# AdaptiveCity/deepdish

Measured on AMD Instinct MI355X. Metric: end-to-end frames/sec (detect+encode+track) at 640x480, higher is better.
Workload: dtype i8 (reference: uint8); encoder f16; 1 GPU; SSD-MobileNet-v1 uint8-quantised (300x300) + MARS-64x32x3 + deep_sort on synthetic 640x480 BGR frames, ~20 synthetic detections/frame (BASELINE.json configs[1]); streams_per_gpu=3072, worker_threads_per_gpu=2, parallelism=independent streams, 3072 per GPU in 2 worker groups, weights=seeded synthetic (seed 1234)

## Files before the change

### deepdish_amd/_lib.py

```python
import ctypes
import os
from ctypes import c_int, c_int64, c_double, c_float, c_void_p, c_char_p, POINTER

HERE = os.path.dirname(os.path.abspath(__file__))
LIB_PATH = os.environ.get('DD_LIB') or os.path.join(HERE, 'libdeepdish_hip.so')

P = c_void_p


class DeepDishHipError(RuntimeError):
    pass


SIGNATURES = {
    'dd_last_error': [],
    'dd_version': [],
    'dd_ctx_create': [c_int, POINTER(P)],
    'dd_ctx_destroy': [P],
    'dd_ctx_stream': [P, POINTER(P)],
    'dd_ctx_sync': [P],
    'dd_kf_initiate': [P, P, P, P, P, c_int, P],
    'dd_kf_predict': [P, P, P, P, c_int, P],
    'dd_kf_project': [P, P, P, P, c_int, P, P, P],
    'dd_kf_update': [P, P, P, P, P, c_int, P],
    'dd_kf_gate': [P, P, P, P, c_int, P, c_int, c_int, P, P],
    'dd_iou_cost': [P, P, P, c_int, P, c_int, P, P],
    'dd_cosine_nn_cost': [P, P, P, c_int, P, c_int, P, P],
    'dd_euclidean_nn_cost': [P, P, P, c_int, P, c_int, P, P],
    'dd_nms': [P, P, P, c_int, c_double, P, P, P],
    'dd_nms_ssd': [P, P, P, c_int, c_double, P, P, P],
    'dd_lsap_host': [P, c_int, c_int, P, P],
    'dd_pyset_difference_order_host': [P, c_int, P, c_int, P, POINTER(c_int)],
    'dd_lsap_batch': [P, P, P, P, P, c_int, P, P],
    'dd_match_cascade': [P, c_int, P, P, c_int, c_int, P, P, c_double, c_double, c_int, P, POINTER(c_int), P, POINTER(c_int), P,
                         POINTER(c_int)],
    'dd_tracker_create': [P, c_double, c_double, c_int, c_int, c_int, c_int, c_int, POINTER(P)],
    'dd_tracker_create_metric': [P, c_int, c_double, c_double, c_int, c_int, c_int, c_int, c_int, POINTER(P)],
    'dd_tracker_destroy': [P],
    'dd_tracker_predict': [P],
    'dd_tracker_update': [P, P, P, c_int, c_int],
    'dd_tracker_count': [P, c_int, POINTER(c_int)],
    'dd_tracker_read': [P, c_int, P, P, P],
    'dd_tracker_track_update': [P, c_int64, P, P, c_int],
    'dd_tracker_track_predict': [P, c_int64],
    'dd_tracker_track_set': [P, c_int64, c_int, c_int],
    'dd_tracker_remove': [P, P, c_int],
    'dd_tracker_next_id': [P, POINTER(c_int64)],
    'dd_tracker_last_cost': [P, P, P, c_int, POINTER(c_int), POINTER(c_int)],
    'dd_tracker_last_matches': [P, P, c_int, POINTER(c_int)],
    'dd_tracker_set_association': [P, c_int],
    'dd_tracker_association_stats': [P, POINTER(ctypes.c_longlong), POINTER(ctypes.c_longlong), POINTER(ctypes.c_longlong),
                                     POINTER(ctypes.c_longlong)],
    'dd_crop_resize': [P, P, c_int, c_int, P, c_int, c_int, c_int, P, P, P],
    'dd_crop_resize_f64': [P, P, c_int, c_int, P, c_int, c_int, c_int, P, P, P],
    'dd_fake_encode': [P, P, c_int, c_int, P, P],
    'dd_resize_lanczos': [P, P, c_int, c_int, c_int, c_int, P, c_int, c_int, P],
    'dd_resize_lanczos_batch': [P, P, c_int, c_int, c_int, c_int, c_int, P, c_int, c_int, P],
    'dd_resize_lanczos_plan': [P, c_int, c_int, c_int, c_int, c_int, c_int, c_int, P, P, P, POINTER(c_int), POINTER(c_int), POINTER(c_int),
                               POINTER(c_int)],
    'dd_letterbox_geometry': [c_int, c_int, c_int, c_int, POINTER(c_int), POINTER(c_int), POINTER(c_int), POINTER(c_int)],
    'dd_resize_lanczos_letterbox': [P, P, c_int, c_int, c_int, c_int, c_int, P, c_int, c_int, c_int, P],
    'dd_resize_lanczos_letterbox_plan': [P, c_int, c_int, c_int, c_int, c_int, c_int, c_int, POINTER(c_int), POINTER(c_int)],
    'dd_resize_bilinear': [P, P, c_int, c_int, c_int, P, c_int, c_int, P],
    'dd_yuv420_to_bgr': [P, P, c_int, c_int, c_int, c_int, c_int, c_int64, c_int64, P, P],
    'dd_yuv422_to_bgr': [P, P, c_int, c_int, c_int, c_int, c_int, c_int64, P, P],
    'dd_ingest_create': [P, c_int, c_int, c_int, c_int, c_int, c_int, c_int, P],
    'dd_ingest_create_format': [P, c_int, c_int, c_int, c_int, c_int, c_int, c_int, c_int, P],
    'dd_ingest_create_jpeg': [P, c_int, c_int, c_int, c_int, c_int, c_int, c_int, c_int64, P],
    'dd_ingest_jpeg_put': [P, c_int, c_int, P, c_int64],
    'dd_ingest_status': [P, c_int, P],
    'dd_ingest_destroy': [P],
    'dd_ingest_host_slot': [P, c_int, P, P],
    'dd_ingest_submit': [P, c_int],
    'dd_ingest_wait_uploaded': [P, c_int],
    'dd_ingest_acquire': [P, c_int, P, P],
    'dd_ingest_release': [P, c_int, P],
    'dd_mog2_create': [P, c_int, c_int, c_int, c_int, c_double, c_int, POINTER(P)],
    'dd_mog2_destroy': [P],
    'dd_mog2_state': [P, c_int, P, P, P, P],
    'dd_mog2_apply': [P, P, c_double, P, P, P],
    'dd_mask_box_count': [P, P, c_int, c_int, c_int, P, P, c_int, P, P],
    'dd_net_create': [P, P, c_int, P, c_int64, c_int, POINTER(P)],
    'dd_net_create_shared': [P, P, c_int, P, c_int64, c_int, POINTER(P)],
    'dd_net_activation_bytes': [P, POINTER(c_int64)],
    'dd_net_destroy': [P],
    'dd_net_forward': [P, P, c_int, P],
    'dd_net_output': [P, c_int, POINTER(P), POINTER(c_int), POINTER(c_int), POINTER(c_int), POINTER(c_int),
                      POINTER(c_int)],
    'dd_net_use_graph': [P, c_int],
    'dd_net_input_size': [P, POINTER(c_int), POINTER(c_int)],
    'dd_net_max_batch': [P, POINTER(c_int)],
    'dd_net_last_batch': [P, POINTER(c_int)],
    'dd_net_read': [P, c_int, c_int, P, c_int, P],
    'dd_net_profile': [P, c_int],
    'dd_net_profile_read': [P, P, c_int, POINTER(c_int)],
    'dd_net_op_launches': [P, P, c_int, POINTER(c_int)],
    'dd_net_op_variants': [P, P, c_int, POINTER(c_int)],
    'dd_netq_dwpw_fits': [c_int, c_int, c_int, c_int, c_int, c_int, POINTER(c_int)],
    'dd_ssd_postprocess': [P, P, P, c_int, c_int, c_int, c_float, c_float, P, P, P, P, P],
    'dd_ssd_decode': [P, P, P, c_int, c_int, c_float, P, P, P, P, c_int, P],
    'dd_ssd_postprocess_decoded': [P, P, P, P, P, c_int, c_int, c_float, c_float, P, P, P, P, c_int, P],
    'dd_ssd_regular_nms_decoded': [P, P, P, c_int, c_int, c_int, c_int, c_int, c_int, c_float, c_float, P, P, P, P, c_int, P],
    'dd_ssd_postprocess_regular': [P, P, P, c_int, c_int, c_int, c_int, c_float, c_float, P, P, P, P, c_int, P],
    'dd_ssd_postprocess_regular_u8': [P, P, P, c_int, P, P, P, c_int, c_int, c_int, c_int, c_float, c_float, P, P, P, P, c_int, P],
    'dd_net_ssd_heads_u8': [P, POINTER(P), POINTER(P), POINTER(c_int), POINTER(P), P, POINTER(c_int), POINTER(c_int)],
    'dd_net_ssd_decode': [P, P, c_int, c_float, c_int],
    'dd_net_ssd_decoded': [P, POINTER(P), POINTER(P), POINTER(P), POINTER(P)],
# ... 83 lines not shown
```

### deepdish_amd/csrc/image.hip

```cpp
#include <cmath>
#include <cstdlib>
#include <map>
#include <mutex>
#include <tuple>
#include <vector>
#include <algorithm>
#include <cstdint>
#include "common.h"
#include "resize_dev.h"
#include "lanczos_tab.h"

namespace {

constexpr int PRECISION_BITS = 32 - 8 - 2;

__global__ __launch_bounds__(256) void crop_resize_k(const uint8_t *__restrict__ frames, int H, int W,
                                                     const CropBox *__restrict__ boxes, int oh, int ow,
                                                     uint8_t *__restrict__ out) {
    const int p = blockIdx.x * blockDim.x + threadIdx.x;
    if (p >= oh * ow) return;
    const CropBox b = boxes[blockIdx.y];
    uint8_t *o = out + ((size_t)blockIdx.y * oh * ow + p) * 3;
    if (b.cw <= 0) { o[0] = o[1] = o[2] = 0; return; }
    const int dy = p / ow, dx = p - dy * ow;
// ... 760 lines not shown
        return DD_OK;
    });
    if (rc != DD_OK) return rc;
    const dim3 grid((unsigned)(bh.n_slabs * batch));
#define DD_LF(KH_, KV_) hipLaunchKernelGGL((lanczos_fused_k<KH_, KV_>), grid, dim3(256), lf_lds_bytes(), s, src, src_img_stride, H, pitch_s, bh.start, \
                                           bh.slab_u0, static_cast<const i4v *>(bh.coef), bh.bias, bh.n_groups, bh.n_cols, bv.start,                 \
                                           static_cast<const i4v *>(bv.coef), bv.bias, bv.n_groups, h, dst, dst_img_stride, bh.n_slabs)
    if (bh.ksteps == 1) DD_LF(1, 1);
    else DD_LF(2, 1);
#undef DD_LF
    DD_LAUNCH_CHECK();
    return DD_OK;
}

}

namespace ddk {

struct LanczosPlan { int h_step = DD_LANCZOS_H_NONE, v_step = DD_LANCZOS_V_NONE, h_ksteps = 0, v_ksteps = 0; };

int crop_box_host(const int64_t *b, int ph, int pw, int H, int W, int *sx, int *sy, int *cw, int *ch) {
    int64_t x = b[0], y = b[1], w = b[2], h = b[3];
    const double aspect = (double)pw / ph;
    const double new_width = aspect * (double)h;
    x = (int64_t)((double)x - (new_width - (double)w) / 2);
    w = (int64_t)new_width;
    int64_t x2 = x + w, y2 = y + h;
    if (x < 0) x = 0;
    if (y < 0) y = 0;
    if (x2 > W - 1) x2 = W - 1;
    if (y2 > H - 1) y2 = H - 1;
    if (x >= x2 || y >= y2) { *sx = *sy = 0; *cw = *ch = 0; return 0; }
    *sx = (int)x; *sy = (int)y; *cw = (int)(x2 - x); *ch = (int)(y2 - y);
    return 1;
}

int crop_box_host_f64(const double *b, int ph, int pw, int H, int W, int *sx, int *sy, int *cw, int *ch) {
    double x = b[0], y = b[1], w = b[2], h = b[3];
    const double new_width = (double)pw / ph * h;
    x -= (new_width - w) / 2;
    w = new_width;
    const double xe = x + w, ye = y + h;
    if (!(fabs(x) < 9e15 && fabs(y) < 9e15 && fabs(xe) < 9e15 && fabs(ye) < 9e15)) { *sx = *sy = 0; *cw = *ch = 0; return 0; }
    int64_t x1 = (int64_t)x, y1 = (int64_t)y, x2 = (int64_t)xe, y2 = (int64_t)ye;
    if (x1 < 0) x1 = 0;
    if (y1 < 0) y1 = 0;
    if (x2 > W - 1) x2 = W - 1;
    if (y2 > H - 1) y2 = H - 1;
    if (x1 >= x2 || y1 >= y2) { *sx = *sy = 0; *cw = *ch = 0; return 0; }
    *sx = (int)x1; *sy = (int)y1; *cw = (int)(x2 - x1); *ch = (int)(y2 - y1);
    return 1;
}

int crop_resize(hipStream_t s, const uint8_t *frames, int H, int W, const void *d_boxes, int n, int oh, int ow,
                uint8_t *out) {
    if (n <= 0) return DD_OK;
    static const bool quad_off = getenv("DD_CROP_QUADS") && atoi(getenv("DD_CROP_QUADS")) == 0;
    if (!quad_off && ow % 4 == 0 && (reinterpret_cast<uintptr_t>(out) & 3) == 0)
        hipLaunchKernelGGL(crop_resize4_k, dim3(dd_ceil_div(oh * (ow / 4), 256), n), dim3(256), 0, s, frames, H, W,
                           static_cast<const CropBox *>(d_boxes), oh, ow, out);
    else
    hipLaunchKernelGGL(crop_resize_k, dim3(dd_ceil_div(oh * ow, 256), n), dim3(256), 0, s, frames, H, W,
                       static_cast<const CropBox *>(d_boxes), oh, ow, out);
    DD_LAUNCH_CHECK();
    return DD_OK;
}

int lanczos_plan(int device, const void *src, int H, int W, int src_c, int swap_rb, const void *dst, int h, int w, const void *tmp,
                 int batch, LanczosPlan *pl) {
    (void)batch;
    static const int dbg = getenv("DD_LANCZOS_DEBUG") ? atoi(getenv("DD_LANCZOS_DEBUG")) : 0;
    static const bool fused_off = getenv("DD_LANCZOS_FUSED") && atoi(getenv("DD_LANCZOS_FUSED")) == 0;
    static const bool no_wide = getenv("DD_LANCZOS_NO_WIDE") != nullptr;
    const uintptr_t a_src = reinterpret_cast<uintptr_t>(src), a_dst = reinterpret_cast<uintptr_t>(dst), a_tmp = reinterpret_cast<uintptr_t>(tmp);
    *pl = LanczosPlan();
    if (!(dbg & 4) && w != W && h != H && (src_c == 3 || src_c == 4) && (W * src_c) % 16 == 0 && H % 16 == 0 &&
        (w * 3) % 4 == 0 && (a_src & 15) == 0 && (a_tmp & 15) == 0 && (a_dst & 3) == 0 && ((size_t)H * W * src_c) % 16 == 0) {
        BandTable bh, bv;
        int rc = get_band(device, W, w, 0, src_c, swap_rb, W * src_c, false, &bh);
        if (rc != DD_OK) return rc;
        rc = get_band(device, H, h, 1, 1, 0, H, false, &bv);
        if (rc != DD_OK) return rc;
        if (bh.ok && bv.ok) {
            pl->h_ksteps = bh.ksteps;
            pl->v_ksteps = bv.ksteps;
            if (!fused_off && bh.ksteps <= 2 && bv.ksteps == 1 && bv.n_groups <= 4 * LF_NVG && H <= 512 && bh.slab_width <= 256 && W * src_c >= 256) {
                pl->h_step = DD_LANCZOS_H_FUSED;
                pl->v_step = DD_LANCZOS_V_FUSED;
            } else {
                pl->h_step = !no_wide && band_wide_ok(H, tmp, (size_t)w * 3 * H, H) ? DD_LANCZOS_H_BAND_WIDE : DD_LANCZOS_H_BAND_NARROW;
                pl->v_step = !no_wide && band_wide_ok(w * 3, dst, (size_t)h * w * 3, w * 3) ? DD_LANCZOS_V_BAND_WIDE : DD_LANCZOS_V_BAND_NARROW;
            }
            return DD_OK;
        }
    }
    const void *mid = src;
    if (w != W) {
        pl->h_step = (!(dbg & 1) && (W * src_c) % 16 == 0 && (a_src & 15) == 0 && W * src_c <= 6144 && lanczos_ksize(W, w) <= HTAPS) ? DD_LANCZOS_H_ROW
                                                                                                                       : DD_LANCZOS_H_SCALAR;
        mid = (h != H) ? tmp : dst;
    } else if (src_c != 3 || swap_rb) {
        const void *o = (h != H) ? tmp : dst;
        pl->h_step = (src_c == 3 && swap_rb && (H * W) % 4 == 0 && ((a_src | reinterpret_cast<uintptr_t>(o)) & 3) == 0) ? DD_LANCZOS_H_SWAP_COPY
                                                                                                                        : DD_LANCZOS_H_COPY;
        mid = o;
    }
    if (h != H)
        pl->v_step = (!(dbg & 2) && (w * 3) % 4 == 0 && (reinterpret_cast<uintptr_t>(mid) & 3) == 0 && (a_dst & 3) == 0) ? DD_LANCZOS_V_V4
                                                                                                                         : DD_LANCZOS_V_SCALAR;
    else if (mid != dst)
        pl->v_step = DD_LANCZOS_V_MEMCPY;
// ... 69 lines not shown
            break;
    }
    return DD_OK;
}

}

extern "C" {

int dd_crop_resize(dd_ctx *ctx, const uint8_t *frame, int H, int W, const int64_t *boxes_host, int n, int ph,
                   int pw, uint8_t *out, int *valid_host, void *stream) {
    DD_REQUIRE(ctx && n >= 0 && H > 0 && W > 0 && ph > 0 && pw > 0, DD_E_ARG, "dd_crop_resize: bad argument");
    DD_DEVICE(ctx);
    if (n == 0) return DD_OK;
    DD_REQUIRE(frame && boxes_host && out, DD_E_ARG, "dd_crop_resize: NULL argument");
    hipStream_t s = dd_pick_stream(ctx, stream);
    int rc;
    if ((rc = ctx->pin[1].reserve((size_t)n * 32)) != DD_OK) return rc;
    if ((rc = ctx->scratch[3].reserve((size_t)n * 32)) != DD_OK) return rc;
    int *hb = ctx->pin[1].as<int>();
    for (int i = 0; i < n; ++i) {
        const int ok = ddk::crop_box_host(boxes_host + (size_t)i * 4, ph, pw, H, W, hb + 8 * i, hb + 8 * i + 1,
                                          hb + 8 * i + 2, hb + 8 * i + 3);
        hb[8 * i + 4] = 0; hb[8 * i + 5] = 0; hb[8 * i + 6] = 0; hb[8 * i + 7] = 0;
        if (valid_host) valid_host[i] = ok;
    }
    DD_HIP(hipMemcpyAsync(ctx->scratch[3].p, hb, (size_t)n * 32, hipMemcpyHostToDevice, s));
    DD_HIP(hipStreamSynchronize(s));
    return ddk::crop_resize(s, frame, H, W, ctx->scratch[3].p, n, ph, pw, out);
}

int dd_crop_resize_f64(dd_ctx *ctx, const uint8_t *frame, int H, int W, const double *boxes_host, int n, int ph,
                       int pw, uint8_t *out, int *valid_host, void *stream) {
    DD_REQUIRE(ctx && n >= 0 && H > 0 && W > 0 && ph > 0 && pw > 0, DD_E_ARG, "dd_crop_resize_f64: bad argument");
    DD_DEVICE(ctx);
    if (n == 0) return DD_OK;
    DD_REQUIRE(frame && boxes_host && out, DD_E_ARG, "dd_crop_resize_f64: NULL argument");
    hipStream_t s = dd_pick_stream(ctx, stream);
    int rc;
    if ((rc = ctx->pin[1].reserve((size_t)n * 32)) != DD_OK) return rc;
    if ((rc = ctx->scratch[3].reserve((size_t)n * 32)) != DD_OK) return rc;
    int *hb = ctx->pin[1].as<int>();
    for (int i = 0; i < n; ++i) {
        const int ok = ddk::crop_box_host_f64(boxes_host + (size_t)i * 4, ph, pw, H, W, hb + 8 * i, hb + 8 * i + 1,
                                              hb + 8 * i + 2, hb + 8 * i + 3);
        hb[8 * i + 4] = 0; hb[8 * i + 5] = 0; hb[8 * i + 6] = 0; hb[8 * i + 7] = 0;
        if (valid_host) valid_host[i] = ok;
    }
    DD_HIP(hipMemcpyAsync(ctx->scratch[3].p, hb, (size_t)n * 32, hipMemcpyHostToDevice, s));
    DD_HIP(hipStreamSynchronize(s));
    return ddk::crop_resize(s, frame, H, W, ctx->scratch[3].p, n, ph, pw, out);
}

int dd_fake_encode(dd_ctx *ctx, const uint8_t *patches, int n, int mode, float *out, void *stream) {
    DD_REQUIRE(ctx && n >= 0 && (mode == 0 || mode == 1), DD_E_ARG, "dd_fake_encode: bad argument");
    DD_DEVICE(ctx);
    if (n == 0) return DD_OK;
    DD_REQUIRE(out && (mode == 1 || patches), DD_E_ARG, "dd_fake_encode: NULL argument");
    hipLaunchKernelGGL(fake_encode_k, dim3(dd_ceil_div(n, 4)), dim3(256), 0, dd_pick_stream(ctx, stream), patches, n, mode, out);
    DD_LAUNCH_CHECK();
    return DD_OK;
}

int dd_resize_lanczos(dd_ctx *ctx, const uint8_t *src, int H, int W, int src_c, int swap_rb, uint8_t *dst, int h,
                      int w, void *stream) {
    DD_REQUIRE(ctx && src && dst && H > 0 && W > 0 && h > 0 && w > 0, DD_E_ARG, "dd_resize_lanczos: bad argument");
    DD_DEVICE(ctx);
    DD_REQUIRE(src_c == 3 || src_c == 4, DD_E_ARG, "dd_resize_lanczos: src_c must be 3 or 4");
    int rc;
    if ((rc = ctx->scratch[3].reserve((size_t)H * w * 3 + 64)) != DD_OK) return rc;
    return ddk::resize_lanczos(dd_pick_stream(ctx, stream), ctx->device, src, H, W, src_c, swap_rb, dst, h, w,
                               ctx->scratch[3].as<uint8_t>(), 1);
}

int dd_resize_lanczos_plan(dd_ctx *ctx, int H, int W, int src_c, int swap_rb, int h, int w, int batch, const void *src, const void *dst,
                           const void *tmp, int *h_step, int *v_step, int *h_ksteps, int *v_ksteps) {
    DD_REQUIRE((ctx || tmp) && batch > 0 && H > 0 && W > 0 && h > 0 && w > 0, DD_E_ARG, "dd_resize_lanczos_plan: bad argument");
    DD_REQUIRE(src_c == 3 || src_c == 4, DD_E_ARG, "dd_resize_lanczos_plan: src_c must be 3 or 4");
    if (!tmp) {
        DD_DEVICE(ctx);
        int rc;
        if ((rc = ctx->scratch[3].reserve((size_t)batch * H * w * 3 + 64)) != DD_OK) return rc;
        tmp = ctx->scratch[3].p;
    }
    ddk::LanczosPlan pl;
    const int rc = ddk::lanczos_plan(ctx ? ctx->device : 0, src, H, W, src_c, swap_rb, dst, h, w, tmp, batch, &pl);
    if (rc != DD_OK) return rc;
    if (h_step) *h_step = pl.h_step;
    if (v_step) *v_step = pl.v_step;
    if (h_ksteps) *h_ksteps = pl.h_ksteps;
    if (v_ksteps) *v_ksteps = pl.v_ksteps;
    return DD_OK;
}

int dd_resize_lanczos_batch(dd_ctx *ctx, const uint8_t *src, int batch, int H, int W, int src_c, int swap_rb, uint8_t *dst,
                            int h, int w, void *stream) {
    DD_REQUIRE(ctx && src && dst && batch > 0 && H > 0 && W > 0 && h > 0 && w > 0, DD_E_ARG, "dd_resize_lanczos_batch: bad argument");
    DD_DEVICE(ctx);
    DD_REQUIRE(src_c == 3 || src_c == 4, DD_E_ARG, "dd_resize_lanczos_batch: src_c must be 3 or 4");
    int rc;
    if ((rc = ctx->scratch[3].reserve((size_t)batch * H * w * 3 + 64)) != DD_OK) return rc;
    return ddk::resize_lanczos(dd_pick_stream(ctx, stream), ctx->device, src, H, W, src_c, swap_rb, dst, h, w,
                               ctx->scratch[3].as<uint8_t>(), batch);
}

int dd_resize_bilinear(dd_ctx *ctx, const uint8_t *src, int H, int W, int c, uint8_t *dst, int h, int w,
// ... 17 lines not shown
```

### deepdish_amd/csrc/netsq.hip

```cpp
#include <algorithm>
#include <atomic>
#include <cstdlib>
#include <type_traits>
#include "common.h"
#include "ssd_dev.h"
#include "net_priv.h"
#include "netsq_dev.h"

namespace {


struct QConvP {
    const uint8_t *in; int H, W, c16_in;
    int kh, kw, stride, off_y, off_x;
    int ho, wo, m;
    const i4v *w;
    const int *cbias;
    int kc_per_tap, n_mfrag, mq;
    uint8_t *out; int epi;
    int Ho, Wo, c16_out;
    long long img_bytes_out; int row_bytes, base_off, cout_store;
    int zwc;
    unsigned hw_magic, wo_magic;
    QReq R;
// ... 370 lines not shown
#pragma unroll
    for (int f = 0; f < 4; ++f) {
        int q = (fg * 4 + f) * 16 + fr;
        live[f] = q < P.m;
        q = min(q, P.m - 1);
        int n, y;
        if (P.hw_magic) { n = (int)__umulhi((unsigned)q, P.hw_magic); y = (int)__umulhi((unsigned)(q - n * hw), P.wo_magic); }
        else { n = q / hw; y = (q - n * hw) / P.wo; }
        const int r = q - n * hw, x = r - y * P.wo;
        src[f] = P.in + (size_t)((unsigned)(n * (P.H + 2) + y * P.stride + P.off_y) * RP + (unsigned)cg * PP + (unsigned)(x * P.stride + P.off_x) * 16u);
        dst[f] = P.out + (size_t)((unsigned)((n * (P.ho + 2) + y + 1) * P.c16 + cg) * PPo + (unsigned)(x + 1) * 16u + 4u * (unsigned)fq);
    }
    i4v acc[4];
#pragma unroll
    for (int f = 0; f < 4; ++f) acc[f] = cbv;
    i4v b[3][4];
#pragma unroll
    for (int ks = 0; ks < 3; ++ks) {
        const int tp = min(4 * ks + fq, 8);
        const unsigned to = (unsigned)(tp / 3) * RP + (unsigned)(tp % 3) * 16u;
#pragma unroll
        for (int f = 0; f < 4; ++f) b[ks][f] = *reinterpret_cast<const i4v *>(src[f] + to);
    }
#pragma unroll
    for (int ks = 0; ks < 3; ++ks) {
        const unsigned sel = 0x01010101u * (unsigned)ks;
        const unsigned rh = __builtin_amdgcn_perm(ab.x, ab.x, sel), rl = __builtin_amdgcn_perm(ab.y, ab.y, sel);
        i4v Ah, Al;
#pragma unroll
        for (int d = 0; d < 4; ++d) { Ah[d] = (int)(rh & dmask[d]); Al[d] = (int)(rl & dmask[d]); }
#pragma unroll
        for (int f = 0; f < 4; ++f) acc[f] = __builtin_amdgcn_mfma_i32_16x16x64_i8(Ah, b[ks][f], acc[f], 0, 0, 0);
#pragma unroll
        for (int f = 0; f < 4; ++f) acc[f] = __builtin_amdgcn_mfma_i32_16x16x64_i8(Al, b[ks][f], acc[f], 0, 0, 0);
    }
    const int M = P.R.M, sh = P.R.e - 1, lo = P.R.lo, hi = P.R.hi;
    const long long C = P.R.C;
#pragma unroll
    for (int f = 0; f < 4; ++f) {
        const unsigned packed = 0x80808080u ^ q_requant_pack4<SAT ? 1 : 0>(acc[f][0], acc[f][1], acc[f][2], acc[f][3], M, C, C, C, C, sh, lo, hi);
        if (live[f]) *reinterpret_cast<unsigned *>(dst[f]) = packed;
    }
}

struct QDecP {
    const uint8_t *box, *cls;
    int n_anchors, n_classes, cls_stride;
    const uint8_t *lut;
    float box_scale, box_zp, sc_scale, sc_zp, thr;
    const float *anchors;
    float *boxes, *score, *keys; int *cls_out;
};

__global__ __launch_bounds__(256) void q_ssd_decode_k(const QDecP P) {
    __shared__ uint8_t lut[256];
    lut[threadIdx.x] = P.lut[threadIdx.x];
    __syncthreads();
    const int a = (blockIdx.x * 256 + threadIdx.x) >> 3, sub = threadIdx.x & 7;
    const size_t z = blockIdx.y;
    const bool live = a < P.n_anchors;
    const uint8_t *c = P.cls + (z * P.n_anchors + (live ? a : 0)) * P.cls_stride;
    int best = -1, bi = 0x7fffffff;
    if (sub * 16 < P.n_classes) {
        const u4v v = *reinterpret_cast<const u4v *>(c + sub * 16);
#pragma unroll
        for (int i = 0; i < 16; ++i) {
            const int k = sub * 16 + i;
            const int q = lut[(v[i >> 2] >> (8 * (i & 3))) & 0xffu];
            if (k >= 1 && k < P.n_classes && q > best) { best = q; bi = k - 1; }
        }
    }
#pragma unroll
    for (int o = 4; o > 0; o >>= 1) {
        const int ob = __shfl_xor(best, o, 64), oi = __shfl_xor(bi, o, 64);
        if (ob > best || (ob == best && oi < bi)) { best = ob; bi = oi; }
    }
    if (live && sub == 0) {
#pragma clang fp contract(off)
        const uint8_t *b = P.box + (z * P.n_anchors + a) * 4;
        float r[4], an[4], bx[4];
#pragma unroll
        for (int q = 0; q < 4; ++q) { r[q] = P.box_scale * ((float)b[q] - P.box_zp); an[q] = P.anchors[a * 4 + q]; }
        (void)ssddev::decode_anchor(r, an, 0.f, bx);
        const float sc = P.sc_scale * ((float)best - P.sc_zp);
        const size_t o = z * P.n_anchors + a;
#pragma unroll
        for (int q = 0; q < 4; ++q) P.boxes[o * 4 + q] = bx[q];
        P.score[o] = sc;
        P.cls_out[o] = bi;
        P.keys[o] = sc >= P.thr ? sc : -1.f;
    }
}

struct QDwpwP {
    const uint8_t *in; int H, W;
    int off_y, off_x, ho, wo, hw, tiles_per_frame;
    uint8_t *out; int c16_out;
    const uint2 *dw_a;
    const long long *dw_cq;
    const i4v *w;
    const i4v *w2;
    const int *cbias;
    const long long *cq;
    int zwc, NR;
    int dup;
    unsigned wo_magic, nr_magic, tpf_magic;
    unsigned long long *dbg;
    QReq Rd, Rp;
};

constexpr int QT = 64;

template <int CIN, int COUT, int WP, int STRIDE, int LPT, bool ROWSUM, int MW = 4, int SAT = 0, bool HL = false, int QTT = QT>
__global__ __launch_bounds__((COUT / (16 * MW)) * WP * 64, (COUT / (16 * MW)) * WP <= 2 ? 3 : QTT > 64 ? 4 : 2) void q_dwpw_k(const QDwpwP P, const int n_tiles, const int tiles_per_block) {
    constexpr int WM = COUT / (16 * MW), NW = WM * WP, NT = NW * 64;
    static_assert(MW == 4 || MW == 2, "fragments per wave");
    static_assert(!(HL && ROWSUM), "the split filter needs no row sums");
    constexpr int KC = (CIN + 63) / 64, CINP = KC * 64, C16 = CIN / 16;
    constexpr int FPT = QTT / 16, UNITS = C16 * (FPT / 4);
    static_assert(QTT % 64 == 0 && UNITS % NW == 0, "depthwise units over waves");
    constexpr int CPW = UNITS / NW;
    static_assert(FPT == 4 || CPW == 1, "several units per wave: one fragment quad only");
    constexpr bool KEEP = CPW <= 2, FOLDP = !ROWSUM && KC <= 4 && QTT == 64;
    extern __shared__ __attribute__((aligned(16))) uint8_t smem[];
    const int tid = threadIdx.x, lane = tid & 63, wave = __builtin_amdgcn_readfirstlane(tid >> 6);
    const int fr = lane & 15, fq = lane >> 4;
    const int wm = wave / WP, wp = wave % WP;
    const int RB = (P.W + 2) * CIN, PP = (P.W + 2) * 16;
    uint8_t *opnd = smem;
    int *rowsum = reinterpret_cast<int *>(opnd + QTT * CINP);
    i4v *pinfo = reinterpret_cast<i4v *>(rowsum + 2 * QTT);
    int *cbl = reinterpret_cast<int *>(pinfo + 2 * QTT);
    uint2 *dwa_l = reinterpret_cast<uint2 *>(cbl + COUT);
    long long *dwq_l = reinterpret_cast<long long *>(dwa_l + (KEEP ? 0 : C16 * 64));
    uint8_t *ring = reinterpret_cast<uint8_t *>(dwq_l + (KEEP ? 0 : CIN));

    i4v Wr[MW][KC];
#pragma unroll
    for (int m = 0; m < MW; ++m)
#pragma unroll
        for (int kc = 0; kc < KC; ++kc) Wr[m][kc] = P.w[((size_t)(wm * MW + m) * KC + kc) * 64 + lane];
    const int mg = (wm * MW) / 4, m0 = (wm * MW) % 4;
    unsigned wlm = 0;
    int kcl = -1;
// ... 1017 lines not shown
                       "dd_net_forward: uint8 block %d: shapes / multipliers the fused kernel does not take", i);
            const long long in_img = (long long)(P.H + 2) * (P.W + 2) * ts->cs, out_img = (long long)(P.ho + 2) * (P.wo + 2) * td->cs;
            const long long lim = 4294967295ll / out_img, n_chunks = (nimg + lim - 1) / lim, chunk = (nimg + n_chunks - 1) / n_chunks;
            DD_REQUIRE(lim >= 1, DD_E_CAPACITY, "dd_net_forward: uint8 block %d: one frame's output beyond 32-bit offsets", i);
            const int dev = net->ctx->device;
            for (long long c0 = 0; c0 < nimg; c0 += chunk) {
                const int nc = (int)std::min(chunk, nimg - c0);
                QDwpwP Q = P;
                Q.in = P.in + c0 * in_img; Q.out = P.out + c0 * out_img;
                bool ok = false;
                int v = 0;
                const int rc = dwpw_dispatch(s, Q, nc, dev, cin, cout, stride, &ok, false, &v);
                if (rc != DD_OK) return rc;
                if (ok) *variant = v | (int)std::min(n_chunks, 127ll) << 21;
                DD_REQUIRE(ok, DD_E_ARG, "dd_net_forward: uint8 block %d (%d -> %d, stride %d, %d x %d): no fused kernel for this shape -- compile the program with the two-op form", i, cin, cout, stride, P.H, P.W);
            }
            return DD_OK;
        }
        case OP_QADD: {
            DD_REQUIRE(ts && td && o[3] >= 0 && o[3] < (int)net->tensors.size(), DD_E_ARG, "dd_net_forward: uint8 ADD %d: operands", i);
            const TensorDesc *tb = &net->tensors[o[3]];
            QAddP P;
            P.A = make_add(o);
            DD_REQUIRE(ts->pad == 1 && td->pad == 1 && tb->pad == 1 && ts->h == td->h && ts->w == td->w && ts->cs == td->cs && tb->h == td->h && tb->w == td->w &&
                       tb->cs == td->cs && td->cs % 16 == 0 && dst != src && dst != o[3] && add_ok(P.A), DD_E_ARG, "dd_net_forward: uint8 ADD %d: tensor layouts / parameters", i);
            P.H = td->h; P.W = td->w; P.c16 = td->cs / 16;
            const long long per_img = (long long)P.H * P.c16 * P.W, img_bytes = (long long)(P.H + 2) * (P.W + 2) * td->cs;
            DD_REQUIRE(per_img < (1ll << 31) - 256, DD_E_CAPACITY, "dd_net_forward: uint8 ADD %d: one frame beyond 31-bit items", i);
            const long long chunk = ((1ll << 31) - 256) / per_img;
            for (long long c0 = 0; c0 < nimg; c0 += chunk) {
                const long long nc = std::min(chunk, nimg - c0);
                P.a = base(src) + c0 * img_bytes; P.b = base(o[3]) + c0 * img_bytes; P.out = base(dst) + c0 * img_bytes;
                P.n_items = (int)(nc * per_img);
                *variant = QV_ADD | (int)std::min((nimg + chunk - 1) / chunk, 255ll) << 8;
                hipLaunchKernelGGL(q_add_k, dim3((unsigned)dd_ceil_div(P.n_items, 256)), dim3(256), 0, s, P);
                DD_LAUNCH_CHECK();
            }
            if (i < (int)net->op_launch.size()) net->op_launch[i] = 22;
            return DD_OK;
        }
        case OP_QSSD_DECODE: {
            if (!net->ssd_dec) return DD_OK;
            QDecP P;
            const TensorDesc &tb = net->tensors[o[1]], &tc = net->tensors[o[3]];
            P.box = base(o[1]); P.cls = base(o[3]);
            P.n_anchors = o[21]; P.n_classes = o[20]; P.cls_stride = tc.cs;
            DD_REQUIRE(P.n_anchors == net->dec_anchors && tb.cs == 4 && tb.h == P.n_anchors && tc.h == P.n_anchors && P.n_classes <= tc.cs, DD_E_ARG,
                       "dd_net_forward: uint8 decode of %d anchors, set up for %d", P.n_anchors, net->dec_anchors);
            P.lut = reinterpret_cast<const uint8_t *>(W + (size_t)(uint32_t)o[16]);
            const float *of = reinterpret_cast<const float *>(o);
            P.box_scale = of[32]; P.box_zp = of[33]; P.sc_scale = of[34]; P.sc_zp = of[35]; P.thr = net->dec_thr;
            P.anchors = net->d_anchors; P.boxes = net->dec_boxes; P.score = net->dec_score; P.keys = net->dec_keys; P.cls_out = net->dec_cls;
            DD_REQUIRE(P.cls_stride % 16 == 0 && P.n_classes <= 128, DD_E_ARG, "dd_net_forward: uint8 decode: %d classes in rows of %d bytes", P.n_classes, P.cls_stride);
            *variant = QV_DECODE;
            hipLaunchKernelGGL(q_ssd_decode_k, dim3(dd_ceil_div(P.n_anchors * 8, 256), nimg), dim3(256), 0, s, P);
            DD_LAUNCH_CHECK();
            return DD_OK;
        }
        default:
            DD_REQUIRE(false, DD_E_ARG, "dd_net_forward: uint8 op kind %d at %d is not built", kind, i);
    }
    return DD_OK;
}
```

### include/deepdish_hip.h

```cpp
#ifndef DEEPDISH_HIP_H
#define DEEPDISH_HIP_H

#include <stdint.h>

#ifdef __cplusplus
extern "C" {
#endif

#define DD_OK            0
#define DD_E_ARG        -1
#define DD_E_HIP        -2
#define DD_E_STATE      -3
#define DD_E_CAPACITY   -4

#define DD_FEATURE_DIM 128

typedef struct dd_ctx dd_ctx;
typedef struct dd_tracker dd_tracker;
typedef struct dd_net dd_net;
typedef struct dd_pipeline dd_pipeline;

const char *dd_last_error(void);
int dd_version(void);

// ... 21 lines not shown
                      const float *feats, int n_d, double *out, void *stream);

int dd_euclidean_nn_cost(dd_ctx *ctx, const float *gallery, const int *offsets_host, int n_t,
                         const float *feats, int n_d, double *out, void *stream);

int dd_nms(dd_ctx *ctx, const double *tlwh, const double *keys, int k, double max_overlap,
           int *out_idx, int *out_n, void *stream);

int dd_nms_ssd(dd_ctx *ctx, const double *xyxy, const double *scores, int k, double iou_thr,
               int *out_idx, int *out_n, void *stream);

int dd_lsap_host(const double *cost_host, int nr, int nc, int *row_ind_host, int *col_ind_host);

int dd_pyset_difference_order_host(const int *a_host, int na, const int *b_host, int nb, int *out_host,
                                   int *out_n_host);

#define DD_ASSOC_DEVICE_MAX 256
int dd_lsap_batch(dd_ctx *ctx, const double *cost_dev, const int *nr_host, const int *nc_host, const int64_t *offset_host,
                  int n_problems, int *rows_host, int *cols_host);

int dd_match_cascade(dd_ctx *ctx, int where, const double *app, const double *iou, int T, int n, const int *state_host,
                     const int *tsu_host, double max_cos, double max_iou, int max_age, int *matches_host, int *n_matches_host,
                     int *un_rows_host, int *n_un_rows_host, int *un_dets_host, int *n_un_dets_host);

int dd_tracker_create(dd_ctx *ctx, double max_cosine_distance, double max_iou_distance,
                      int max_age, int n_init, int nn_budget ,
                      int track_capacity, int gallery_capacity, dd_tracker **out);
int dd_tracker_create_metric(dd_ctx *ctx, int metric, double matching_threshold, double max_iou_distance,
                             int max_age, int n_init, int nn_budget ,
                             int track_capacity, int gallery_capacity, dd_tracker **out);
int dd_tracker_destroy(dd_tracker *trk);
int dd_tracker_predict(dd_tracker *trk);
int dd_tracker_update(dd_tracker *trk, const double *tlwh_host, const float *feats,
                      int feats_on_device, int n);
int dd_tracker_count(dd_tracker *trk, int which, int *out_n_host);
int dd_tracker_read(dd_tracker *trk, int which, int64_t *ints6_host, double *means_host,
                    double *covs_host);
int dd_tracker_track_update(dd_tracker *t, int64_t track_id, const double *tlwh_host, const float *feat, int feat_on_device);
int dd_tracker_track_predict(dd_tracker *t, int64_t track_id);
int dd_tracker_track_set(dd_tracker *t, int64_t track_id, int state, int time_since_update);
int dd_tracker_remove(dd_tracker *t, const int64_t *track_ids_host, int n);
int dd_tracker_next_id(dd_tracker *trk, int64_t *out_host);

int dd_tracker_last_cost(dd_tracker *trk, double *app_host, double *iou_host, int cap, int *rows_host, int *cols_host);
int dd_tracker_last_matches(dd_tracker *trk, int *pairs_host, int cap, int *out_m_host);
int dd_tracker_set_association(dd_tracker *trk, int where);
int dd_tracker_association_stats(dd_tracker *trk, long long *device_updates_host, long long *host_updates_host,
                                 long long *fallback_streams_host, long long *d2h_bytes_host);

int dd_crop_resize(dd_ctx *ctx, const uint8_t *frame, int H, int W, const int64_t *boxes_host,
                   int n, int ph, int pw, uint8_t *out, int *valid_host, void *stream);
int dd_crop_resize_f64(dd_ctx *ctx, const uint8_t *frame, int H, int W, const double *boxes_host, int n, int ph,
                       int pw, uint8_t *out, int *valid_host, void *stream);

int dd_fake_encode(dd_ctx *ctx, const uint8_t *patches, int n, int mode, float *out, void *stream);

int dd_resize_lanczos(dd_ctx *ctx, const uint8_t *src, int H, int W, int src_c, int swap_rb,
                      uint8_t *dst, int h, int w, void *stream);
int dd_resize_lanczos_batch(dd_ctx *ctx, const uint8_t *src, int batch, int H, int W, int src_c, int swap_rb,
                            uint8_t *dst, int h, int w, void *stream);
#define DD_LANCZOS_H_NONE 0
#define DD_LANCZOS_H_COPY 1
#define DD_LANCZOS_H_SWAP_COPY 2
#define DD_LANCZOS_H_ROW 3
#define DD_LANCZOS_H_SCALAR 4
#define DD_LANCZOS_H_BAND_WIDE 5
#define DD_LANCZOS_H_BAND_NARROW 6
#define DD_LANCZOS_H_FUSED 7
#define DD_LANCZOS_V_NONE 0
#define DD_LANCZOS_V_MEMCPY 1
#define DD_LANCZOS_V_V4 2
#define DD_LANCZOS_V_SCALAR 3
#define DD_LANCZOS_V_BAND_WIDE 4
#define DD_LANCZOS_V_BAND_NARROW 5
#define DD_LANCZOS_V_FUSED 6
int dd_resize_lanczos_plan(dd_ctx *ctx, int H, int W, int src_c, int swap_rb, int h, int w, int batch, const void *src,
                           const void *dst, const void *tmp, int *h_step, int *v_step, int *h_ksteps, int *v_ksteps);
int dd_letterbox_geometry(int W, int H, int net_w, int net_h, int *new_w, int *new_h, int *off_x, int *off_y);
int dd_resize_lanczos_letterbox(dd_ctx *ctx, const uint8_t *src, int batch, int H, int W, int src_c, int swap_rb, uint8_t *dst, int h, int w,
                                int pad, void *stream);
int dd_resize_lanczos_letterbox_plan(dd_ctx *ctx, int H, int W, int src_c, int swap_rb, int h, int w, int batch, int *path, int *rows_per_block);
int dd_resize_bilinear(dd_ctx *ctx, const uint8_t *src, int H, int W, int c,
                       uint8_t *dst, int h, int w, void *stream);

int dd_yuv420_to_bgr(dd_ctx *ctx, const uint8_t *src, int batch, int H, int W, int layout, int pitch, int64_t chroma_offset,
                     int64_t frame_stride, uint8_t *dst, void *stream);
int dd_yuv422_to_bgr(dd_ctx *ctx, const uint8_t *src, int batch, int H, int W, int order, int pitch, int64_t frame_stride, uint8_t *dst,
                     void *stream);

typedef struct dd_ingest dd_ingest;
typedef struct dd_jpegdec dd_jpegdec;
int dd_ingest_create(dd_ctx *ctx, int slots, int n_streams, int src_h, int src_w, int dst_h, int dst_w, int flip,
                     dd_ingest **out);
int dd_ingest_create_format(dd_ctx *ctx, int slots, int n_streams, int src_h, int src_w, int dst_h, int dst_w, int flip,
                            int pixel_format, dd_ingest **out);
int dd_ingest_create_jpeg(dd_ctx *ctx, int slots, int n_streams, int src_h, int src_w, int dst_h, int dst_w, int flip, int64_t slot_bytes,
                          dd_ingest **out);
int dd_ingest_jpeg_put(dd_ingest *g, int slot, int stream, const uint8_t *data_host, int64_t n);
int dd_ingest_status(dd_ingest *g, int slot, int *status_host);
int dd_ingest_destroy(dd_ingest *g);
int dd_ingest_host_slot(dd_ingest *g, int slot, uint8_t **host_ptr, int64_t *n_bytes);
int dd_ingest_wait_uploaded(dd_ingest *g, int slot);
int dd_ingest_submit(dd_ingest *g, int slot);
int dd_ingest_acquire(dd_ingest *g, int slot, void *consumer_stream, const uint8_t **frames_dev);
int dd_ingest_release(dd_ingest *g, int slot, void *consumer_stream);

// ... 175 lines not shown
```

Measured before the change: 145,100 frames/s.

## Add fast uint8 SSD decode using monotone LUT byte-max argmax

Adds a new uint8 SSD decode kernel that handles four anchors per 8-lane group. When the dequant LUT is monotone, it takes the raw byte maximum across class lanes and finds the first matching index with SWAR byte-equality tricks, instead of a LUT lookup and compare per class. It also vectorises the box and anchor loads and the output store, and falls back to the per-class sweep when the LUT is not monotone. Separately it adds test-facing crop_resize_boxes and crop_resize_kernel entry points, which are unrelated to speed. The decode is a small part of the end-to-end pipeline, and the bit tricks carry a correctness risk on tie handling.

```diff
diff --git a/deepdish_amd/_lib.py b/deepdish_amd/_lib.py
--- a/deepdish_amd/_lib.py
+++ b/deepdish_amd/_lib.py
@@ -53,6 +53,8 @@
                                      POINTER(ctypes.c_longlong)],
     'dd_crop_resize': [P, P, c_int, c_int, P, c_int, c_int, c_int, P, P, P],
     'dd_crop_resize_f64': [P, P, c_int, c_int, P, c_int, c_int, c_int, P, P, P],
+    'dd_crop_resize_boxes': [P, P, c_int, c_int, c_int, P, c_int, c_int, c_int, P, P],
+    'dd_crop_resize_kernel': [c_int, c_int, P, POINTER(c_int)],
     'dd_fake_encode': [P, P, c_int, c_int, P, P],
     'dd_resize_lanczos': [P, P, c_int, c_int, c_int, c_int, P, c_int, c_int, P],
     'dd_resize_lanczos_batch': [P, P, c_int, c_int, c_int, c_int, c_int, P, c_int, c_int, P],
diff --git a/deepdish_amd/csrc/image.hip b/deepdish_amd/csrc/image.hip
--- a/deepdish_amd/csrc/image.hip
+++ b/deepdish_amd/csrc/image.hip
@@ -836,11 +836,15 @@
     return 1;
 }
 
+int crop_kernel_for(int oh, int ow, const void *out) {
+    static const bool quad_off = getenv("DD_CROP_QUADS") && atoi(getenv("DD_CROP_QUADS")) == 0;
+    return !quad_off && ow % 4 == 0 && (reinterpret_cast<uintptr_t>(out) & 3) == 0 ? 1 : 0;
+}
+
 int crop_resize(hipStream_t s, const uint8_t *frames, int H, int W, const void *d_boxes, int n, int oh, int ow,
                 uint8_t *out) {
     if (n <= 0) return DD_OK;
-    static const bool quad_off = getenv("DD_CROP_QUADS") && atoi(getenv("DD_CROP_QUADS")) == 0;
-    if (!quad_off && ow % 4 == 0 && (reinterpret_cast<uintptr_t>(out) & 3) == 0)
+    if (crop_kernel_for(oh, ow, out) == 1)
         hipLaunchKernelGGL(crop_resize4_k, dim3(dd_ceil_div(oh * (ow / 4), 256), n), dim3(256), 0, s, frames, H, W,
                            static_cast<const CropBox *>(d_boxes), oh, ow, out);
     else
@@ -1016,6 +1020,35 @@
     return ddk::crop_resize(s, frame, H, W, ctx->scratch[3].p, n, ph, pw, out);
 }
 
+int dd_crop_resize_boxes(dd_ctx *ctx, const uint8_t *frames, int n_frames, int H, int W, const int32_t *boxes_host, int n, int ph, int pw,
+                         uint8_t *out, void *stream) {
+    DD_REQUIRE(ctx && n >= 0 && n_frames > 0 && H > 0 && W > 0 && ph > 0 && pw > 0, DD_E_ARG, "dd_crop_resize_boxes: bad argument");
+    DD_DEVICE(ctx);
+    if (n == 0) return DD_OK;
+    DD_REQUIRE(frames && boxes_host && out, DD_E_ARG, "dd_crop_resize_boxes: NULL argument");
+    for (int i = 0; i < n; ++i) {
+        const int32_t *b = boxes_host + (size_t)i * 8;
+        DD_REQUIRE(b[2] <= 0 || (b[3] >= 1 && b[0] >= 0 && b[1] >= 0 && (long long)b[0] + b[2] <= W && (long long)b[1] + b[3] <= H && b[4] >= 0 && b[4] < n_frames),
+                   DD_E_ARG, "dd_crop_resize_boxes: box %d (%d, %d, %d x %d, frame %d) is not inside a %d x %d frame of %d", i, b[0], b[1], b[2], b[3], b[4], W, H, n_frames);
+    }
+    hipStream_t s = dd_pick_stream(ctx, stream);
+    int rc;
+    if ((rc = ctx->pin[1].reserve((size_t)n * 32)) != DD_OK) return rc;
+    if ((rc = ctx->scratch[3].reserve((size_t)n * 32)) != DD_OK) return rc;
+    int *hb = ctx->pin[1].as<int>();
+    for (int i = 0; i < n; ++i)
+        for (int k = 0; k < 8; ++k) hb[8 * i + k] = k == 5 || k == 6 ? (boxes_host[(size_t)i * 8 + k] != 0) : k == 7 ? 0 : boxes_host[(size_t)i * 8 + k];
+    DD_HIP(hipMemcpyAsync(ctx->scratch[3].p, hb, (size_t)n * 32, hipMemcpyHostToDevice, s));
+    DD_HIP(hipStreamSynchronize(s));
+    return ddk::crop_resize(s, frames, H, W, ctx->scratch[3].p, n, ph, pw, out);
+}
+
+int dd_crop_resize_kernel(int ph, int pw, const void *out, int *kernel_host) {
+    DD_REQUIRE(ph > 0 && pw > 0 && kernel_host, DD_E_ARG, "dd_crop_resize_kernel: bad argument");
+    *kernel_host = ddk::crop_kernel_for(ph, pw, out);
+    return DD_OK;
+}
+
 int dd_fake_encode(dd_ctx *ctx, const uint8_t *patches, int n, int mode, float *out, void *stream) {
     DD_REQUIRE(ctx && n >= 0 && (mode == 0 || mode == 1), DD_E_ARG, "dd_fake_encode: bad argument");
     DD_DEVICE(ctx);
diff --git a/deepdish_amd/csrc/netsq.hip b/deepdish_amd/csrc/netsq.hip
--- a/deepdish_amd/csrc/netsq.hip
+++ b/deepdish_amd/csrc/netsq.hip
@@ -446,6 +446,44 @@
     float *boxes, *score, *keys; int *cls_out;
 };
 
+__device__ __forceinline__ void q_dec_sweep(const uint8_t *lut, const uint8_t *c, const int sub, const int n_classes, int &best, int &bi) {
+    best = -1; bi = 0x7fffffff;
+    if (sub * 16 < n_classes) {
+        const u4v v = *reinterpret_cast<const u4v *>(c + sub * 16);
+#pragma unroll
+        for (int i = 0; i < 16; ++i) {
+            const int k = sub * 16 + i;
+            const int q = lut[(v[i >> 2] >> (8 * (i & 3))) & 0xffu];
+            if (k >= 1 && k < n_classes && q > best) { best = q; bi = k - 1; }
+        }
+    }
+#pragma unroll
+    for (int o = 4; o > 0; o >>= 1) {
+        const int ob = __shfl_xor(best, o, 64), oi = __shfl_xor(bi, o, 64);
+        if (ob > best || (ob == best && oi < bi)) { best = ob; bi = oi; }
+    }
+}
+
+template <bool VEC = false>
+__device__ __forceinline__ void q_dec_finish(const QDecP &P, const size_t z, const int a, const int best, const int bi, const unsigned bw, const float (&an)[4]) {
+#pragma clang fp contract(off)
+    float r[4], bx[4];
+#pragma unroll
+    for (int q = 0; q < 4; ++q) r[q] = P.box_scale * ((float)((bw >> (8 * q)) & 0xffu) - P.box_zp);
+    (void)ssddev::decode_anchor(r, an, 0.f, bx);
+    const float sc = P.sc_scale * ((float)best - P.sc_zp);
+    const size_t o = z * P.n_anchors + a;
+    if constexpr (VEC) {
+        *reinterpret_cast<float4 *>(P.boxes + o * 4) = float4{bx[0], bx[1], bx[2], bx[3]};
+    } else {
+#pragma unroll
+        for (int q = 0; q < 4; ++q) P.boxes[o * 4 + q] = bx[q];
+    }
+    P.score[o] = sc;
+    P.cls_out[o] = bi;
+    P.keys[o] = sc >= P.thr ? sc : -1.f;
+}
+
 __global__ __launch_bounds__(256) void q_ssd_decode_k(const QDecP P) {
     __shared__ uint8_t lut[256];
     lut[threadIdx.x] = P.lut[threadIdx.x];
@@ -454,36 +492,96 @@
     const size_t z = blockIdx.y;
     const bool live = a < P.n_anchors;
     const uint8_t *c = P.cls + (z * P.n_anchors + (live ? a : 0)) * P.cls_stride;
-    int best = -1, bi = 0x7fffffff;
-    if (sub * 16 < P.n_classes) {
-        const u4v v = *reinterpret_cast<const u4v *>(c + sub * 16);
-#pragma unroll
-        for (int i = 0; i < 16; ++i) {
-            const int k = sub * 16 + i;
-            const int q = lut[(v[i >> 2] >> (8 * (i & 3))) & 0xffu];
-            if (k >= 1 && k < P.n_classes && q > best) { best = q; bi = k - 1; }
-        }
-    }
-#pragma unroll
-    for (int o = 4; o > 0; o >>= 1) {
-        const int ob = __shfl_xor(best, o, 64), oi = __shfl_xor(bi, o, 64);
-        if (ob > best || (ob == best && oi < bi)) { best = ob; bi = oi; }
-    }
+    int best, bi;
+    q_dec_sweep(lut, c, sub, P.n_classes, best, bi);
     if (live && sub == 0) {
-#pragma clang fp contract(off)
         const uint8_t *b = P.box + (z * P.n_anchors + a) * 4;
-        float r[4], an[4], bx[4];
-#pragma unroll
-        for (int q = 0; q < 4; ++q) { r[q] = P.box_scale * ((float)b[q] - P.box_zp); an[q] = P.anchors[a * 4 + q]; }
-        (void)ssddev::decode_anchor(r, an, 0.f, bx);
-        const float sc = P.sc_scale * ((float)best - P.sc_zp);
-        const size_t o = z * P.n_anchors + a;
-#pragma unroll
-        for (int q = 0; q < 4; ++q) P.boxes[o * 4 + q] = bx[q];
-        P.score[o] = sc;
-        P.cls_out[o] = bi;
-        P.keys[o] = sc >= P.thr ? sc : -1.f;
-    }
+        float an[4];
+#pragma unroll
+        for (int q = 0; q < 4; ++q) an[q] = P.anchors[a * 4 + q];
+        q_dec_finish(P, z, a, best, bi, (unsigned)b[0] | (unsigned)b[1] << 8 | (unsigned)b[2] << 16 | (unsigned)b[3] << 24, an);
+    }
+}
+
+constexpr int DEC_NA = 4;
+
+__global__ __launch_bounds__(256) void q_ssd_decode_fast_k(const QDecP P) {
+    __shared__ uint8_t lut[256];
+    __shared__ unsigned first[256];
+    __shared__ unsigned short qt[256];
+    __shared__ int mono;
+    const int tid = threadIdx.x, lane = tid & 63;
+    const int sub = lane & 7, grp = lane >> 3;
+    const int wbase = blockIdx.x * (32 * DEC_NA) + (tid >> 6) * (8 * DEC_NA);
+    const size_t z = blockIdx.y;
+    const int rem = P.n_classes - sub * 16;
+    u4v x[DEC_NA];
+#pragma unroll
+    for (int j = 0; j < DEC_NA; ++j) {
+        const int a = wbase + 8 * j + grp;
+        x[j] = u4v{0u, 0u, 0u, 0u};
+        if (rem > 0) x[j] = *reinterpret_cast<const u4v *>(P.cls + (z * P.n_anchors + (a < P.n_anchors ? a : 0)) * P.cls_stride + sub * 16);
+    }
+    const int af = wbase + lane;
+    const bool fin = lane < 8 * DEC_NA && af < P.n_anchors;
+    unsigned bw = 0u;
+    float an[4] = {0.f, 0.f, 0.f, 0.f};
+    if (fin) {
+        bw = *reinterpret_cast<const unsigned *>(P.box + (z * P.n_anchors + af) * 4);
+        const float4 av = *reinterpret_cast<const float4 *>(P.anchors + (size_t)af * 4);
+        an[0] = av.x; an[1] = av.y; an[2] = av.z; an[3] = av.w;
+    }
+    const unsigned lv = P.lut[tid];
+    lut[tid] = (uint8_t)lv;
+    first[tid] = 256u;
+    if (tid == 0) mono = 1;
+    __syncthreads();
+    atomicMin(&first[lv], (unsigned)tid);
+    if (tid > 0 && lv < lut[tid - 1]) atomicAnd(&mono, 0);
+    __syncthreads();
+    qt[tid] = (unsigned short)(lv | first[lv] << 8);
+    __syncthreads();
+    const bool sweep = !mono || P.n_classes < 2;
+    int fbest = -1, fbi = 0x7fffffff;
+#pragma unroll
+    for (int j = 0; j < DEC_NA; ++j) {
+        const int a = wbase + 8 * j + grp;
+        int best, bi;
+        if (sweep) {
+            q_dec_sweep(lut, P.cls + (z * P.n_anchors + (a < P.n_anchors ? a : 0)) * P.cls_stride, sub, P.n_classes, best, bi);
+        } else {
+            u4v v = x[j];
+            if (rem > 0) {
+#pragma unroll
+                for (int d = 0; d < 4; ++d) {
+                    const int kd = rem - 4 * d;
+                    v[d] &= kd >= 4 ? 0xffffffffu : kd <= 0 ? 0u : (1u << (8 * kd)) - 1u;
+                }
+                if (sub == 0) v[0] &= 0xffffff00u;
+            }
+            unsigned m = 0;
+#pragma unroll
+            for (int d = 0; d < 4; ++d) m = max(max(m, v[d] & 0xffu), max(max((v[d] >> 8) & 0xffu, (v[d] >> 16) & 0xffu), v[d] >> 24));
+#pragma unroll
+            for (int o = 4; o > 0; o >>= 1) m = max(m, (unsigned)__shfl_xor((int)m, o, 64));
+            const unsigned e = qt[m];
+            best = (int)(e & 0xffu);
+            const unsigned t = e >> 8, nb = ~(t * 0x01010101u);
+            unsigned g[4];
+#pragma unroll
+            for (int d = 0; d < 4; ++d) g[d] = ((v[d] | nb) - (((v[d] ^ nb) >> 1) & 0x7f7f7f7fu)) & 0x80808080u;
+            const unsigned long long glo = g[0] | (unsigned long long)g[1] << 32, ghi = g[2] | (unsigned long long)g[3] << 32;
+            int k = 0x7fffffff;
+            if (glo) k = sub * 16 + (__builtin_ctzll(glo) >> 3) - 1;
+            else if (ghi) k = sub * 16 + 8 + (__builtin_ctzll(ghi) >> 3) - 1;
+#pragma unroll
+            for (int o = 4; o > 0; o >>= 1) k = min(k, __shfl_xor(k, o, 64));
+            bi = t == 0u ? 0 : k;
+        }
+        const int tb = __shfl(best, 8 * (lane & 7), 64), ti = __shfl(bi, 8 * (lane & 7), 64);
+        if ((lane >> 3) == j) { fbest = tb; fbi = ti; }
+    }
+    if (fin) q_dec_finish<true>(P, z, af, fbest, fbi, bw, an);
 }
 
 struct QDwpwP {
@@ -1607,8 +1705,10 @@
             P.box_scale = of[32]; P.box_zp = of[33]; P.sc_scale = of[34]; P.sc_zp = of[35]; P.thr = net->dec_thr;
             P.anchors = net->d_anchors; P.boxes = net->dec_boxes; P.score = net->dec_score; P.keys = net->dec_keys; P.cls_out = net->dec_cls;
             DD_REQUIRE(P.cls_stride % 16 == 0 && P.n_classes <= 128, DD_E_ARG, "dd_net_forward: uint8 decode: %d classes in rows of %d bytes", P.n_classes, P.cls_stride);
-            *variant = QV_DECODE;
-            hipLaunchKernelGGL(q_ssd_decode_k, dim3(dd_ceil_div(P.n_anchors * 8, 256), nimg), dim3(256), 0, s, P);
+            static const bool fast_off = getenv("DD_Q_DEC_FAST") && atoi(getenv("DD_Q_DEC_FAST")) == 0;
+            *variant = QV_DECODE | (fast_off ? 0 : 1) << 4;
+            if (!fast_off) hipLaunchKernelGGL(q_ssd_decode_fast_k, dim3(dd_ceil_div(P.n_anchors, 32 * DEC_NA), nimg), dim3(256), 0, s, P);
+            else hipLaunchKernelGGL(q_ssd_decode_k, dim3(dd_ceil_div(P.n_anchors * 8, 256), nimg), dim3(256), 0, s, P);
             DD_LAUNCH_CHECK();
             return DD_OK;
         }
diff --git a/include/deepdish_hip.h b/include/deepdish_hip.h
--- a/include/deepdish_hip.h
+++ b/include/deepdish_hip.h
@@ -97,6 +97,9 @@
                    int n, int ph, int pw, uint8_t *out, int *valid_host, void *stream);
 int dd_crop_resize_f64(dd_ctx *ctx, const uint8_t *frame, int H, int W, const double *boxes_host, int n, int ph,
                        int pw, uint8_t *out, int *valid_host, void *stream);
+int dd_crop_resize_boxes(dd_ctx *ctx, const uint8_t *frames, int n_frames, int H, int W, const int32_t *boxes_host, int n, int ph, int pw,
+                         uint8_t *out, void *stream);
+int dd_crop_resize_kernel(int ph, int pw, const void *out, int *kernel_host);
 
 int dd_fake_encode(dd_ctx *ctx, const uint8_t *patches, int n, int mode, float *out, void *stream);
 
```

Result: no change. 144,500 frames/s (-0.4%).
